# ziotom78/pytracer

Measured on NVIDIA B200. Metric: path-traced rays/sec (demo.txt 1080p), higher is better.
Workload: dtype f32

## Files before the change

pytracer_b200/csrc/rt_warp.cuh:

```cuda
#pragma once
#include "rt_kernels.cuh"

#define RT_WARP_MAX_THREADS 256
#ifndef RT_WARP_SPLIT
#define RT_WARP_SPLIT 1
#endif


struct __align__(16) ScatterRec {
  float4 a;
  float4 b;
  float4 c;
};

struct WarpCfg {
  int cap;
  int group;
  int per_pixel;
  int rounds;
  int per_warp_bytes;
  int shape_bytes;
  long long n_tasks;
  float bg[3], inv_n, inv_spp;
  unsigned n_magic;
  double inv_w, inv_h, inv_s;
  unsigned long long n_samples;
};

RT_DEV int err_batch_of(const ErrArgs& cfg, int ls) {
  return cfg.err_bpp == 32 ? (ls & 31) : ls - (int)(((unsigned)ls * cfg.err_magic) >> 16) * cfg.err_bpp;
}
RT_DEV void err_batch_add(float* bsum, int slot, bool on, V3<float> c, int lane) {
  const unsigned FULL = 0xffffffffu;
  if (__ballot_sync(FULL, on && (c.x != 0.f || c.y != 0.f || c.z != 0.f)) == 0u) return;
  const int key = on ? slot : 32 + lane;
  const int prev = __shfl_up_sync(FULL, key, 1);
  const unsigned heads = __ballot_sync(FULL, lane == 0 || prev != key);
  const int seg_start = 31 - __clz(heads & (0xffffffffu >> (31 - lane)));
#pragma unroll
  for (int d = 1; d < 32; d <<= 1) {
    const float r = __shfl_up_sync(FULL, c.x, d);
    const float g = __shfl_up_sync(FULL, c.y, d);
    const float b = __shfl_up_sync(FULL, c.z, d);
    if (lane - d >= seg_start) { c.x += r; c.y += g; c.z += b; }
  }
  const bool tail = lane == 31 || ((heads >> (lane + 1)) & 1u);
  if (on && tail && (c.x != 0.f || c.y != 0.f || c.z != 0.f)) {
    atomicAdd(&bsum[3 * slot + 0], c.x);
    atomicAdd(&bsum[3 * slot + 1], c.y);
    atomicAdd(&bsum[3 * slot + 2], c.z);
  }
}
RT_DEV void err_store(const ErrArgs& e, int L, const float* bsum, int g, long long entry, V3<float> m, int lane) {
  const unsigned FULL = 0xffffffffu;
  const int bpp = e.err_bpp, B = min(L, bpp);
  float tr = 0.f, tg = 0.f, tb = 0.f;
  if (lane < B) {
    const float n = (float)((L - 1 - lane) / bpp + 1);
    const float* t = bsum + 3 * (g * bpp + lane);
    const float dr = fmaf(-n, m.x, t[0]), dg = fmaf(-n, m.y, t[1]), db = fmaf(-n, m.z, t[2]);
    tr = dr * dr / n; tg = dg * dg / n; tb = db * db / n;
  }
#pragma unroll
  for (int d = 16; d > 0; d >>= 1) {
    tr += __shfl_xor_sync(FULL, tr, d);
    tg += __shfl_xor_sync(FULL, tg, d);
    tb += __shfl_xor_sync(FULL, tb, d);
  }
  if (lane == 0) {
    const float k = 1.f / ((float)(B - 1) * (float)L);
    float* o = e.err_mean + 3 * entry;
    o[0] = m.x; o[1] = m.y; o[2] = m.z;
    float* v = e.err_var + 3 * entry;
    v[0] = tr * k; v[1] = tg * k; v[2] = tb * k;
  }
}

#define RT_SMALL_MAX_SPHERES 8
#define RT_SMALL_MAX_SHAPES 16
#define RT_SMALL_MAX_MATERIALS 16
#define RT_SMALL_MAX_PIGMENTS 32
enum {
  SM_INVM = 0,
  SM_M = SM_INVM + RT_SMALL_MAX_SHAPES * 48,
  SM_ORIG = SM_M + RT_SMALL_MAX_SHAPES * 48,
  SM_SHAPE_MAT = SM_ORIG + RT_SMALL_MAX_SHAPES * 4,
  SM_PIG = SM_SHAPE_MAT + RT_SMALL_MAX_SHAPES * 16,
  SM_PIG_STRIDE = 48,
  SM_BYTES = SM_PIG + RT_SMALL_MAX_PIGMENTS * SM_PIG_STRIDE
};
#ifndef RT_SMALL_THREADS
#define RT_SMALL_THREADS 256
#endif
#ifndef RT_SMALL_MINB
#define RT_SMALL_MINB 3
#endif

RT_DEV void stage_words(void* sh, const void* g, int bytes) {
  const uint32_t* src = reinterpret_cast<const uint32_t*>(g);
  uint32_t* dst = reinterpret_cast<uint32_t*>(sh);
  for (int i = threadIdx.x; i < bytes / 4; i += blockDim.x) dst[i] = __ldg(src + i);
}

RT_DEV float4 lds4(uint32_t a) {
  float4 v;
  asm volatile("ld.shared.v4.f32 {%0, %1, %2, %3}, [%4];" : "=f"(v.x), "=f"(v.y), "=f"(v.z), "=f"(v.w) : "r"(a) : "memory");
  return v;
}
RT_DEV void sts4(uint32_t a, float4 v) {
  asm volatile("st.shared.v4.f32 [%0], {%1, %2, %3, %4};" :: "r"(a), "f"(v.x), "f"(v.y), "f"(v.z), "f"(v.w) : "memory");
}
RT_DEV float4 lds4c(uint32_t a) {
  float4 v;
  asm volatile("ld.shared.v4.f32 {%0, %1, %2, %3}, [%4];" : "=f"(v.x), "=f"(v.y), "=f"(v.z), "=f"(v.w) : "r"(a));
  return v;
}
RT_DEV int4 lds4ic(uint32_t a) {
  int4 v;
  asm volatile("ld.shared.v4.s32 {%0, %1, %2, %3}, [%4];" : "=r"(v.x), "=r"(v.y), "=r"(v.z), "=r"(v.w) : "r"(a));
  return v;
}
RT_DEV int ldsic(uint32_t a) {
  int v;
  asm volatile("ld.shared.s32 %0, [%1];" : "=r"(v) : "r"(a));
  return v;
}
RT_DEV Rows3 lds_rows(uint32_t a) {
  Rows3 m;
  m.r0 = lds4c(a); m.r1 = lds4c(a + 16); m.r2 = lds4c(a + 32);
  return m;
}

RT_DEV void closest_small(uint32_t sb, int n_spheres, int n_shapes, const Ray<float>& r, int origin, float& best_t, int& best) {
  const float inf = Num<float>::inf();
  float ts = inf, tp = inf;
  int is = -1, ip = -1;
  uint32_t a = sb + SM_INVM;
#pragma unroll 1
  for (int i = 0; i < n_spheres; ++i, a += 48) {
    float tm, half;
    bool ok = sphere_cross_rows(lds_rows(a), r, tm, half);
    const float t1 = tm - half;
    float t = (t1 > r.tmin) ? t1 : tm + half;
    if (i == origin) { t = 2.0f * tm; ok = true; }
    if (ok && t > r.tmin && t < ts) { ts = t; is = i; }
  }
#pragma unroll 1
  for (int i = n_spheres; i < n_shapes; ++i, a += 48) {
    const float4 row = lds4c(a + 32);
    const float oz = fmaf(r.o.x, row.x, fmaf(r.o.y, row.y, fmaf(r.o.z, row.z, row.w)));
    const float dz = fmaf(r.d.x, row.x, fmaf(r.d.y, row.y, r.d.z * row.z));
    const float t = -oz * fast_rcp(dz);
    if (!(fabsf(dz) < 1e-5f) && t > r.tmin && t < tp && i != origin) { tp = t; ip = i; }
  }
  bool plane = tp < ts;
  if (tp == ts && ip >= 0 && is >= 0) plane = ldsic(sb + SM_ORIG + 4 * ip) < ldsic(sb + SM_ORIG + 4 * is);
  best_t = plane ? tp : ts;
  best = plane ? ip : is;
}

RT_DEV V3<float> pigment_color_small(uint32_t pa, float u, float v) {
  const int4 h = lds4ic(pa);
  const float4 q = lds4c(pa + 16);
  if (h.x == RT_PIGMENT_UNIFORM) return mk3<float>(q.x, q.y, q.z);
  const float4 w = lds4c(pa + 32);
  if (h.x == RT_PIGMENT_CHECKERED) {
    const int iu = __float2int_rd(u * (float)h.y), iv = __float2int_rd(v * (float)h.y);
    return (((iu ^ iv) & 1) == 0) ? mk3<float>(q.x, q.y, q.z) : mk3<float>(q.w, w.x, w.y);
  }
  int col = (int)(u * (float)h.z), row = (int)(v * (float)h.w);
  col = min(max(col, 0), h.z - 1);
  row = min(max(row, 0), h.w - 1);
  const cudaTextureObject_t tex = ((unsigned long long)__float_as_uint(w.w) << 32) | (unsigned long long)__float_as_uint(w.z);
  const float4 t = fetch_texel(tex, col + 0.5f, row + 0.5f);
  return mk3<float>(t.x, t.y, t.z);
}

RT_DEV Ray<float> primary_ray_mul(const RenderArgs& a, double inv_w, double inv_h, double inv_s, int col, int row, int s, Pcg& aa) {
  double up = 0.5, vp = 0.5;
  if (a.S > 0) {
    const int ir = a.S <= 1024 ? (int)(((float)s + 0.5f) * (float)inv_s) : s / a.S;
    const int ic = s - ir * a.S;
    const double r1 = (double)pcg_random(aa) * (1.0 / 4294967295.0);
    const double r2 = (double)pcg_random(aa) * (1.0 / 4294967295.0);
    up = ((double)ic + r1) * inv_s;
    vp = ((double)ir + r2) * inv_s;
  }
  const double u = ((double)col + up) * inv_w;
  const double v = 1.0 - ((double)row + vp) * inv_h;
  V3<double> o, d;
  camera_fire_f64(a.cam, u, v, o, d);
  Ray<float> r;
  r.o = cast3<float>(o);
  r.d = cast3<float>(d);
  r.tmin = 1.0e-5f;
  r.tmax = Num<float>::inf();
  return r;
}

RT_DEV int own_stratum(const RenderArgs& a, int ls) {
  return (a.part_mode == RT_PART_SPP && a.part_count > 1) ? a.part_rank + ls * a.part_count : ls;
}

enum { ACC_REG = 0, ACC_LANES = 1, ACC_SEG = 2 };
#define RT_ACC_LANES_MAX_GROUP 8

template <bool SHAPES_SMEM, int ACC, bool SMALL, bool ERR = false>
__global__ void __launch_bounds__(SMALL ? RT_SMALL_THREADS : RT_WARP_MAX_THREADS, SMALL ? RT_SMALL_MINB : 2)
k_pt_warp(const __grid_constant__ SceneView<float> sc, const __grid_constant__ RenderArgs a,
          const __grid_constant__ WarpCfg cfg, const __grid_constant__ ErrArgs ea) {
  extern __shared__ __align__(16) unsigned char smem_raw[];
  const unsigned FULL = 0xffffffffu;
  const int warp = threadIdx.x >> 5;
  ScanSrc<float> src = global_src<float>(sc);
  if (SMALL) {
    stage_words(smem_raw + SM_INVM, sc.invm, sc.n_shapes * 48);
    stage_words(smem_raw + SM_M, sc.m, sc.n_shapes * 48);
    stage_words(smem_raw + SM_ORIG, sc.orig, sc.n_shapes * 4);
    for (int i = threadIdx.x; i < sc.n_shapes; i += blockDim.x) {
      const DevMaterial& mt = sc.materials[sc.material[i]];
      reinterpret_cast<int4*>(smem_raw + SM_SHAPE_MAT)[i] = make_int4(mt.brdf_kind, mt.brdf_pigment, mt.emitted_pigment, mt.flags);
    }
    for (int i = threadIdx.x; i < sc.n_pigments; i += blockDim.x) {
      const DevPigment& pg = sc.pigments[i];
      float4* o = reinterpret_cast<float4*>(smem_raw + SM_PIG + i * SM_PIG_STRIDE);
      o[0] = make_float4(__int_as_float(pg.kind), __int_as_float(pg.steps), __int_as_float(pg.tex_w), __int_as_float(pg.tex_h));
      o[1] = make_float4(pg.c1[0], pg.c1[1], pg.c1[2], pg.c2[0]);
      o[2] = make_float4(pg.c2[1], pg.c2[2], __uint_as_float((uint32_t)pg.tex), __uint_as_float((uint32_t)((unsigned long long)pg.tex >> 32)));
    }
    __syncthreads();
  } else if (SHAPES_SMEM) {
    stage_bytes(smem_raw, sc.packed, (size_t)sc.n_pairs * 96 + (size_t)(sc.n_shapes - sc.n_spheres) * 48);
    __syncthreads();
    src.pairs = reinterpret_cast<const float4*>(smem_raw);
    src.planes = reinterpret_cast<const float*>(smem_raw) + 24 * (size_t)sc.n_pairs;
  }
  const int lane0 = threadIdx.x & 31;
  const int lane = __shfl_sync(FULL, lane0, lane0);
  const uint32_t smem0 = (uint32_t)__cvta_generic_to_shared(smem_raw);
  const uint32_t sb = __shfl_sync(FULL, smem0 + (uint32_t)lane0, 0);
  const int wofs = (SMALL ? (int)SM_BYTES : cfg.shape_bytes) + warp * cfg.per_warp_bytes;
  const uint32_t wb = __shfl_sync(FULL, smem0 + (uint32_t)(wofs + lane0), 0);
  const uint32_t curb = wb + (uint32_t)cfg.cap * (uint32_t)sizeof(ScatterRec);
  constexpr bool MULTI_SLOT = ACC != ACC_REG;
  int* slot_rays = reinterpret_cast<int*>(smem_raw + wofs + (size_t)(cfg.cap + 1) * sizeof(ScatterRec));
  float* acc = reinterpret_cast<float*>(slot_rays + 32);
  float* bsum = ACC == ACC_REG ? reinterpret_cast<float*>(slot_rays) : acc + (ACC == ACC_SEG ? 96 : 96 * cfg.group);
  const bool count_rays = a.out_hit != nullptr && a.hit_mode == RT_HIT_RAY_COUNT;

  const PixelMap pm = ERR ? make_pixel_map_list(a, ea) : make_pixel_map(a);
  const int N = a.num_of_rays;
  const int S2 = a.S > 0 ? a.S * a.S : 1;
  const int G = cfg.group, L = cfg.per_pixel;
  auto div_n = [&](int x) -> int { return cfg.n_magic ? (int)(((unsigned)x * cfg.n_magic) >> 16) : (x >= N ? 1 : 0); };
  const float inv_n = cfg.inv_n, inv_spp = cfg.inv_spp;
  unsigned int n_rays = 0;
  bool overflow = false;

  while (true) {
    long long task = 0;
    if (lane == 0) task = (long long)atomicAdd(a.counters + CNT_TASK, 1ull);
    task = __shfl_sync(FULL, task, 0);
    if (task >= cfg.n_tasks) break;
    const long long p0 = task * G;
    uint64_t aa_task = a.aa_state;
    if (ACC == ACC_REG && a.S > 0 && p0 < pm.n_pixels) {
      int col, row;
      if (ERR) locate_listed(pm, ea, p0, col, row);
      else pm.locate(p0, col, row);
      aa_task = pcg_jump(a.aa_state, 2ull * (unsigned long long)((long long)row * a.width + col) * S2, a.jump);
    }
    float sr = 0.f, sg = 0.f, sb_ = 0.f;
    unsigned int task_rays = 0;
    const int task_prims = (int)min((long long)G, pm.n_pixels - p0) * L;
    if (MULTI_SLOT) {
      if (ACC == ACC_SEG) { for (int i = lane; i < 96; i += 32) acc[i] = 0.f; }
      else { for (int i = 0; i < 3 * cfg.group; ++i) acc[i * 32 + lane] = 0.f; }
      slot_rays[lane] = 0;
      __syncwarp();
    }
    if (ERR) {
      for (int i = lane; i < 96; i += 32) bsum[i] = 0.f;
      __syncwarp();
    }

    {
      int top = 0, cur_rem = 0, cur_done = 0;
      int round = 0;
      bool primary_phase = true;
      while (true) {
        bool active;
        int slot = 0, depth = 0, seg_start = lane, origin = -1;
        V3<float> thr = mk3<float>(1.f, 1.f, 1.f);
        Ray<float> ray;
        Pcg rng;
        long long pix = 0;
        bool last_of_pixel = false;
        int rslot = 0;
        if (primary_phase) {
          const int j = round * 32 + lane;
          slot = j / L;
          const int ls = j - slot * L;
          const long long p = p0 + slot;
          if (ERR) rslot = slot * ea.err_bpp + err_batch_of(ea, ls);
          active = (j < G * L) && (p < pm.n_pixels);
          task_rays += (unsigned)min(max(task_prims - round * 32, 0), 32);
          if (active) {
            int col, row;
            if (ERR) locate_listed(pm, ea, p, col, row);
            else pm.locate(p, col, row);
            pix = (long long)row * a.width + col;
            const int s = own_stratum(a, ls);
            const unsigned long long k = (unsigned long long)pix * S2 + s;
            Pcg aa;
            aa.inc = a.aa_inc;
            if (ACC == ACC_REG) aa.state = (a.S > 0) ? pcg_jump(aa_task, 2ull * (unsigned)s, a.jump) : 0;
            else aa.state = (a.S > 0) ? pcg_jump(a.aa_state, 2ull * k, a.jump) : 0;
            ray = primary_ray_mul(a, cfg.inv_w, cfg.inv_h, cfg.inv_s, col, row, s, aa);
            rng = pcg_seed(a.pt_state, (a.pt_inc >> 1) + k);
            last_of_pixel = (ls == L - 1);
          }
          if (ACC == ACC_SEG) seg_start = max(0, slot * L - round * 32);
        } else {
          const long long avail = (long long)cur_rem + (long long)top * N;
          if (avail == 0) break;
          const int take = (int)min(avail, 32ll);
          active = lane < take;
          task_rays += (unsigned)take;
          const int from_cur = min(cur_rem, take);
          const int jj = max(lane - from_cur, 0);
          const int r = div_n(jj);
          const bool on_cur = lane < from_cur;
          const int child = on_cur ? cur_done + lane : jj - r * N;
          if (ACC == ACC_SEG) seg_start = on_cur ? 0 : from_cur + r * N;
          const uint32_t ra = (on_cur || !active) ? curb : wb + (uint32_t)(top - 1 - r) * (uint32_t)sizeof(ScatterRec);
          ScatterRec rec;
          rec.a = lds4(ra); rec.b = lds4(ra + 16); rec.c = lds4(ra + 32);
          const int rest = take - from_cur;
          const int full = div_n(rest), part = rest - full * N;
          cur_rem -= from_cur;
          cur_done += from_cur;
          __syncwarp();
          int new_top = top - full;
          if (part > 0) {
            new_top -= 1;
            if (lane < 3) sts4(curb + 16 * lane, lds4(wb + (uint32_t)new_top * (uint32_t)sizeof(ScatterRec) + 16 * lane));
            cur_rem = N - part;
            cur_done = part;
          }
          __syncwarp();
          top = new_top;
          if (active) {
            const int meta = __float_as_int(rec.a.w);
            slot = meta & 31;
            if (ERR) { rslot = slot; slot = (int)(((unsigned)rslot * ea.err_magic) >> 16); }
            depth = (meta >> 6) & 1023;
            origin = (int)((unsigned)meta >> 16);
            if (origin == 0xFFFF) origin = -1;
            thr = mk3<float>(rec.b.w, rec.c.x, rec.c.y);
            const uint64_t base = ((uint64_t)__float_as_uint(rec.c.w) << 32) | (uint64_t)__float_as_uint(rec.c.z);
            rng.state = child_stream(base, child);
            rng.inc = a.pt_inc;
            ray.o = mk3<float>(rec.a.x, rec.a.y, rec.a.z);
            ray.tmax = Num<float>::inf();
            const V3<float> nd = mk3<float>(rec.b.x, rec.b.y, rec.b.z);
            if (((meta >> 5) & 1) == RT_BRDF_DIFFUSE) {
              const float u1 = unit_from_u32((uint32_t)(rng.state >> 32));
              const float u2 = unit_from_u32((uint32_t)rng.state);
              ray.d = diffuse_dir<float>(nd, u1, u2);
              ray.tmin = 1.0e-3f;
            } else {
              ray.d = nd;
              ray.tmin = 1e-5f;
            }
          }
        }

        V3<float> contrib = mk3<float>(0.f, 0.f, 0.f);
        bool push = false;
        ScatterRec out;
        float best_t = Num<float>::inf();
        int best = -1;
        if (!SMALL && RT_WARP_SPLIT) {
          if (!active) { ray.o = mk3<float>(0.f, 0.f, 0.f); ray.d = mk3<float>(0.f, 0.f, 0.f); ray.tmin = 0.f; ray.tmax = 0.f; }
          closest_all_warp(sc, src, ray, active, best_t, best, origin);
        }
        if (active) {
          if (SMALL) closest_small(sb, sc.n_spheres, sc.n_shapes, ray, origin, best_t, best);
          else if (!RT_WARP_SPLIT) closest_all_f32<true>(sc, src, ray, best_t, best, origin);
          const bool found = best >= 0;
          if (count_rays) {
            if (MULTI_SLOT) atomicAdd(&slot_rays[slot], 1);
          } else if (primary_phase) {
            if (last_of_pixel && a.out_hit)
              a.out_hit[pm.compact ? p0 + slot : pix] = !found ? -1 : (SMALL ? ldsic(sb + SM_ORIG + 4 * best) : sc.orig[best]);
          }
          if (!found) {
            contrib = mk3<float>(thr.x * cfg.bg[0], thr.y * cfg.bg[1], thr.z * cfg.bg[2]);
          } else {
            int brdf_kind, brdf_pig, emit_pig, mf;
            Rows3 im;
            const bool sphere = best < sc.n_spheres;
            if (SMALL) {
              const int4 mt = lds4ic(sb + SM_SHAPE_MAT + 16 * best);
              brdf_kind = mt.x; brdf_pig = mt.y; emit_pig = mt.z; mf = mt.w;
            } else {
              const DevMaterial& mat = sc.materials[sc.material[best]];
              brdf_kind = mat.brdf_kind; brdf_pig = mat.brdf_pigment; emit_pig = mat.emitted_pigment; mf = mat.flags;
            }
            auto rows_of = [&](bool inverse) -> Rows3 {
              if (SMALL) return lds_rows(sb + (inverse ? SM_INVM : SM_M) + 48 * best);
              return rows_at((inverse ? sc.invm : sc.m) + 12 * (size_t)best);
            };
            auto pig_uniform = [&](int idx) -> V3<float> {
              if (SMALL) { const float4 q = lds4c(sb + SM_PIG + idx * SM_PIG_STRIDE + 16); return mk3<float>(q.x, q.y, q.z); }
              return pig_c1<float>(sc.pigments[idx]);
            };
            auto pig_at = [&](int idx, float u, float v) -> V3<float> {
              if (SMALL) return pigment_color_small(sb + SM_PIG + idx * SM_PIG_STRIDE, u, v);
              return pigment_color<float>(sc.pigments, idx, u, v);
            };
            float u = 0.f, v = 0.f;
            if (depth >= a.max_depth) {
              if (!(mf & MAT_EMIT_BLACK)) {
                if (mf & MAT_UV_EMIT) local_uv<float>(local_hit_rows(rows_of(true), ray, best_t), sphere, u, v);
                contrib = mul3(thr, (mf & MAT_UV_EMIT) ? pig_at(emit_pig, u, v) : pig_uniform(emit_pig));
              }
            } else {
              const bool scatters = !(mf & MAT_NO_SCATTER);
              LocalHit<float> lh;
              if (scatters || (mf & MAT_USES_UV)) { im = rows_of(true); lh = local_hit_rows(im, ray, best_t); }
              if (mf & MAT_USES_UV) local_uv<float>(lh, sphere, u, v);
              if (!(mf & MAT_EMIT_BLACK))
                contrib = mul3(thr, (mf & MAT_UV_EMIT) ? pig_at(emit_pig, u, v) : pig_uniform(emit_pig));
              if (scatters) {
                V3<float> hit_color = (mf & MAT_UV_BRDF) ? pig_at(brdf_pig, u, v) : pig_uniform(brdf_pig);
                const float lum = max3(hit_color);
                bool go_on = true;
                if (depth >= a.rr_limit) {
                  const float q = fmaxf(0.05f, 1.f - lum);
                  if (pcg_random_float<float>(rng) > q) hit_color = fast_rcp(1.f - q) * hit_color;
                  else go_on = false;
                }
                if (go_on && lum > 0.f) {
                  push = true;
                  V3<float> point, normal;
                  world_frame_rows(im, rows_of(false), lh, sphere, point, normal);
                  const V3<float> nd = (brdf_kind == RT_BRDF_DIFFUSE) ? normal : specular_dir<float>(ray.d, normal);
                  const V3<float> w = inv_n * mul3(thr, hit_color);
                  out.a = make_float4(point.x, point.y, point.z,
                                      __int_as_float((ERR ? rslot : slot) | (brdf_kind << 5) | ((depth + 1) << 6) |
                                                     ((best < 0xFFFF ? best : 0xFFFF) << 16)));
                  out.b = make_float4(nd.x, nd.y, nd.z, w.x);
                  out.c = make_float4(w.y, w.z, __uint_as_float((uint32_t)rng.state), __uint_as_float((uint32_t)(rng.state >> 32)));
                }
              }
            }
          }
        }

        if (ERR) err_batch_add(bsum, rslot, active, contrib, lane);
        if (ACC == ACC_SEG) {
#pragma unroll
          for (int d = 1; d < 32; d <<= 1) {
            const float r = __shfl_up_sync(FULL, contrib.x, d);
            const float g = __shfl_up_sync(FULL, contrib.y, d);
            const float b = __shfl_up_sync(FULL, contrib.z, d);
            if (lane - d >= seg_start) { contrib.x += r; contrib.y += g; contrib.z += b; }
          }
          const int next_start = __shfl_down_sync(FULL, seg_start, 1);
          const bool tail = (lane == 31) || (next_start != seg_start);
          if (active && tail && (contrib.x != 0.f || contrib.y != 0.f || contrib.z != 0.f)) {
            atomicAdd(&acc[3 * slot + 0], contrib.x);
            atomicAdd(&acc[3 * slot + 1], contrib.y);
            atomicAdd(&acc[3 * slot + 2], contrib.z);
          }
        } else if (ACC == ACC_LANES) {
          if (active) {
            float* col = acc + (3 * slot) * 32 + lane;
            col[0] += contrib.x; col[32] += contrib.y; col[64] += contrib.z;
          }
        } else {
          sr += contrib.x; sg += contrib.y; sb_ += contrib.z;
        }

        const unsigned pmask = __ballot_sync(FULL, push);
        const int npush = __popc(pmask);
        if (top + npush > cfg.cap) {
          overflow = true;
        } else {
          if (push) {
            const uint32_t pa = wb + (uint32_t)(top + __popc(pmask & ((1u << lane) - 1u))) * (uint32_t)sizeof(ScatterRec);
            sts4(pa, out.a); sts4(pa + 16, out.b); sts4(pa + 32, out.c);
          }
          top += npush;
        }
        __syncwarp();
        if (primary_phase && ++round >= cfg.rounds) primary_phase = false;
      }
    }
    n_rays += task_rays;

    if (ERR && ACC == ACC_SEG) {
      __syncwarp();
      for (int g = 0; g < G && p0 + g < pm.n_pixels; ++g)
        err_store(ea, L, bsum, g, p0 + g, mk3<float>(acc[3 * g] * inv_spp, acc[3 * g + 1] * inv_spp, acc[3 * g + 2] * inv_spp), lane);
      __syncwarp();
    } else if (ACC == ACC_SEG) {
      __syncwarp();
      const long long p = p0 + lane;
      if (lane < G && p < pm.n_pixels) {
        int col, row;
        pm.locate(p, col, row);
        store_pixel<float>(a, pm.at(p, col, row),
                           mk3<float>(acc[3 * lane] * inv_spp, acc[3 * lane + 1] * inv_spp, acc[3 * lane + 2] * inv_spp));
        if (count_rays) a.out_hit[pm.at(p, col, row)] = slot_rays[lane];
      }
      __syncwarp();
    } else if (ACC == ACC_LANES) {
      __syncwarp();
      for (int g = 0; g < G; ++g) {
        float r = acc[(3 * g) * 32 + lane], gr = acc[(3 * g + 1) * 32 + lane], b = acc[(3 * g + 2) * 32 + lane];
#pragma unroll
        for (int d = 16; d > 0; d >>= 1) {
          r += __shfl_xor_sync(FULL, r, d);
          gr += __shfl_xor_sync(FULL, gr, d);
          b += __shfl_xor_sync(FULL, b, d);
        }
        const long long p = p0 + g;
        if (ERR) {
          if (p < pm.n_pixels) err_store(ea, L, bsum, g, p, mk3<float>(r * inv_spp, gr * inv_spp, b * inv_spp), lane);
        } else if (lane == 0 && p < pm.n_pixels) {
          int col, row;
          pm.locate(p, col, row);
          store_pixel<float>(a, pm.at(p, col, row), mk3<float>(r * inv_spp, gr * inv_spp, b * inv_spp));
          if (count_rays) a.out_hit[pm.at(p, col, row)] = slot_rays[g];
        }
      }
      __syncwarp();
    } else {
#pragma unroll
      for (int d = 16; d > 0; d >>= 1) {
        sr += __shfl_xor_sync(FULL, sr, d);
        sg += __shfl_xor_sync(FULL, sg, d);
        sb_ += __shfl_xor_sync(FULL, sb_, d);
      }
      if (ERR) {
        if (p0 < pm.n_pixels) {
          __syncwarp();
          err_store(ea, L, bsum, 0, p0, mk3<float>(sr * inv_spp, sg * inv_spp, sb_ * inv_spp), lane);
        }
        __syncwarp();
      } else if (lane == 0 && p0 < pm.n_pixels) {
        int col, row;
        pm.locate(p0, col, row);
        store_pixel<float>(a, pm.at(p0, col, row), mk3<float>(sr * inv_spp, sg * inv_spp, sb_ * inv_spp));
        if (count_rays) a.out_hit[pm.at(p0, col, row)] = (int)task_rays;
      }
    }
  }
  if (overflow) atomicExch(a.counters + CNT_OVERFLOW, 1ull);
  if (lane == 0 && n_rays) atomicAdd(a.counters + CNT_CLOSEST, (unsigned long long)n_rays);
  if (blockIdx.x == 0 && threadIdx.x == 0) atomicAdd(a.counters + CNT_SAMPLES, cfg.n_samples);
}

template <bool ERR = false>
inline cudaError_t launch_pt_warp_impl(const SceneView<float>& sc, const RenderArgs& a, cudaStream_t st,
                                       int sm_count, LaunchInfo* info, const char** why_not, ErrArgs ea = ErrArgs()) {
  PixelMap pm = ERR ? make_pixel_map_list(a, ea) : make_pixel_map(a);
  const int S2 = a.S > 0 ? a.S * a.S : 1;
  int L = S2;
  if (a.part_mode == RT_PART_SPP && a.part_count > 1)
    L = a.part_rank < S2 ? (S2 - a.part_rank + a.part_count - 1) / a.part_count : 0;
  if (pm.n_pixels == 0 || L == 0) return cudaSuccess;
  if (a.num_of_rays < 1) { *why_not = "num_of_rays must be >= 1"; return cudaErrorInvalidValue; }
  if (a.max_depth >= 1023) { *why_not = "max_depth >= 1023 is not supported by the warp variant (use mega)"; return cudaErrorInvalidValue; }
  WarpCfg cfg;
  cfg.per_pixel = L;
  size_t shape_bytes = (size_t)sc.n_pairs * 96 + (size_t)(sc.n_shapes - sc.n_spheres) * 48;
  const bool shapes_smem = shape_bytes > 0 && shape_bytes <= 64 * 1024;
  const bool small = sc.n_shapes > 0 && sc.n_spheres <= RT_SMALL_MAX_SPHERES && sc.n_shapes <= RT_SMALL_MAX_SHAPES &&
                     sc.n_materials <= RT_SMALL_MAX_MATERIALS && sc.n_pigments <= RT_SMALL_MAX_PIGMENTS;
  int want = 32;
#ifdef RT_TUNING
  if (const char* env = getenv("RT_WARP_WANT")) want = std::min(std::max(atoi(env), 1), 256);
#endif
  if (L >= 32) cfg.group = 1;
  else if (L >= 4) cfg.group = (want + L - 1) / L < RT_ACC_LANES_MAX_GROUP ? (want + L - 1) / L : RT_ACC_LANES_MAX_GROUP;
  else cfg.group = 32 / L;
  if (cfg.group * L > 32 && !small) cfg.group = 32 / L > 0 ? 32 / L : 1;
  cfg.rounds = (cfg.group * L + 31) / 32;
  cfg.n_tasks = (pm.n_pixels + cfg.group - 1) / cfg.group;
  const long long prims = (long long)cfg.rounds * 32;
  long long cap = a.num_of_rays == 1 ? prims + 32 : prims + 32ll * (long long)a.max_depth;
  if (cap < 64) cap = 64;
  int acc_mode = cfg.group == 1 ? ACC_REG : (cfg.group <= RT_ACC_LANES_MAX_GROUP ? ACC_LANES : ACC_SEG);
  cfg.shape_bytes = small ? (int)SM_BYTES : (shapes_smem ? (int)((shape_bytes + 15) / 16 * 16) : 0);
  const size_t limit = 200 * 1024;
  int warps = (small ? RT_SMALL_THREADS : RT_WARP_MAX_THREADS) / 32;
  size_t per_warp = 0, smem = 0;
  bool with_err = false;
  auto footprint = [&](int mode, int w, size_t& pw) {
    pw = (size_t)(cap + 1) * sizeof(ScatterRec);
    if (mode == ACC_SEG) pw += 32 * sizeof(int) + 96 * sizeof(float);
    if (mode == ACC_LANES) pw += 32 * sizeof(int) + (size_t)cfg.group * 96 * sizeof(float);
    if (with_err) pw += 96 * sizeof(float);
    return cfg.shape_bytes + pw * w;
  };
  if (acc_mode == ACC_LANES) {
    size_t pw_l, pw_s;
    const size_t sm_bytes = 227 * 1024;
    const size_t blocks_lanes = sm_bytes / (footprint(ACC_LANES, warps, pw_l) + 1024);
    const size_t blocks_seg = sm_bytes / (footprint(ACC_SEG, warps, pw_s) + 1024);
    const size_t by_threads = 2048 / (warps * 32), by_regs = small ? RT_SMALL_MINB : 2;
    if (std::min(std::min(blocks_seg, by_threads), by_regs) > std::min(std::min(blocks_lanes, by_threads), by_regs)) acc_mode = ACC_SEG;
#ifdef RT_TUNING
    if (const char* env = getenv("RT_WARP_ACC")) { const int m = atoi(env); if (m == ACC_LANES || m == ACC_SEG) acc_mode = m; }
#endif
  }
  with_err = ERR;
  for (;; warps >>= 1) {
    smem = footprint(acc_mode, warps, per_warp);
    if (smem <= limit || warps == 1) break;
  }
  if (smem > limit) { *why_not = "max_depth needs a deeper work stack than shared memory holds"; return cudaErrorInvalidValue; }
  cfg.cap = (int)cap;
  cfg.per_warp_bytes = (int)per_warp;
  for (int k = 0; k < 3; ++k) cfg.bg[k] = (float)a.background[k];
  cfg.inv_n = 1.0f / (float)a.num_of_rays;
  cfg.inv_spp = 1.0f / (float)S2;
  cfg.n_magic = a.num_of_rays <= 1024 ? (65536u + (unsigned)a.num_of_rays - 1u) / (unsigned)a.num_of_rays : 0u;
  cfg.n_samples = (unsigned long long)pm.n_pixels * (unsigned long long)L;
  cfg.inv_w = 1.0 / (double)a.width;
  cfg.inv_h = 1.0 / (double)a.height;
  cfg.inv_s = a.S > 0 ? 1.0 / (double)a.S : 1.0;
  ea.err_bpp = 32 / cfg.group;
  ea.err_magic = (65536u + (unsigned)ea.err_bpp - 1u) / (unsigned)ea.err_bpp;
  if (ERR && (a.S < 2 || cfg.group > RT_ACC_LANES_MAX_GROUP || L != S2)) {
    *why_not = "the error map needs samples_per_side >= 2 and no partition";
    return cudaErrorInvalidValue;
  }

  void (*kern)(const SceneView<float>, const RenderArgs, const WarpCfg, const ErrArgs);
#define RT_PICK(ACCM)                                                                   \
  (small ? k_pt_warp<true, ACCM, true, ERR> : (shapes_smem ? k_pt_warp<true, ACCM, false, ERR> : k_pt_warp<false, ACCM, false, ERR>))
  if (acc_mode == ACC_REG) kern = RT_PICK(ACC_REG);
  else if (acc_mode == ACC_LANES) kern = RT_PICK(ACC_LANES);
  else kern = RT_PICK(ACC_SEG);
#undef RT_PICK
  cudaError_t e = cudaFuncSetAttribute(kern, cudaFuncAttributeMaxDynamicSharedMemorySize, (int)limit);
  if (e != cudaSuccess) return e;
  int per_sm = 0;
  e = cudaOccupancyMaxActiveBlocksPerMultiprocessor(&per_sm, kern, warps * 32, smem);
  if (e != cudaSuccess) return e;
  if (per_sm < 1) per_sm = 1;
  long long blocks = (long long)per_sm * sm_count;
  long long needed = (cfg.n_tasks + warps - 1) / warps;
  if (blocks > needed) blocks = needed;
  kern<<<(unsigned)blocks, warps * 32, smem, st>>>(sc, a, cfg, ea);
  if (info) { info->n_launches += 1; info->variant = RT_VARIANT_WARP; }
  return cudaGetLastError();
}
```

Before: 66.87 billion.

## Precompute per-lane PCG jump tables in smem and unroll small-scene intersection loops

For the small-scene register-accumulation path, each block precomputes per-lane PCG jump coefficients (mult, plus) into shared memory at setup. Each primary ray then derives its AA RNG state with one multiply-add from a per-round base jump, instead of a full logarithmic pcg_jump per ray. The sphere and plane intersection loops are also fully unrolled to their compile-time maximums with early breaks, removing loop-carried address arithmetic. This uses more shared memory per block and a longer unrolled body, which may raise register pressure. The correctness of the jump composition depends on the stratum mapping being linear in the lane index.

```diff
diff --git a/pytracer_b200/csrc/rt_warp.cuh b/pytracer_b200/csrc/rt_warp.cuh
--- a/pytracer_b200/csrc/rt_warp.cuh
+++ b/pytracer_b200/csrc/rt_warp.cuh
@@ -87,7 +87,9 @@
   SM_SHAPE_MAT = SM_ORIG + RT_SMALL_MAX_SHAPES * 4,
   SM_PIG = SM_SHAPE_MAT + RT_SMALL_MAX_SHAPES * 16,
   SM_PIG_STRIDE = 48,
-  SM_BYTES = SM_PIG + RT_SMALL_MAX_PIGMENTS * SM_PIG_STRIDE
+  SM_BYTES = SM_PIG + RT_SMALL_MAX_PIGMENTS * SM_PIG_STRIDE,
+  SM_JUMP = SM_BYTES,
+  SM_JUMP_BYTES = 32 * 16
 };
 #ifndef RT_SMALL_THREADS
 #define RT_SMALL_THREADS 256
@@ -125,6 +127,11 @@
   asm volatile("ld.shared.s32 %0, [%1];" : "=r"(v) : "r"(a));
   return v;
 }
+RT_DEV ulonglong2 lds2u64c(uint32_t a) {
+  ulonglong2 v;
+  asm volatile("ld.shared.v2.u64 {%0, %1}, [%2];" : "=l"(v.x), "=l"(v.y) : "r"(a));
+  return v;
+}
 RT_DEV Rows3 lds_rows(uint32_t a) {
   Rows3 m;
   m.r0 = lds4c(a); m.r1 = lds4c(a + 16); m.r2 = lds4c(a + 32);
@@ -135,24 +142,28 @@
   const float inf = Num<float>::inf();
   float ts = inf, tp = inf;
   int is = -1, ip = -1;
-  uint32_t a = sb + SM_INVM;
-#pragma unroll 1
-  for (int i = 0; i < n_spheres; ++i, a += 48) {
+#pragma unroll
+  for (int i = 0; i < RT_SMALL_MAX_SPHERES; ++i) {
+    if (i >= n_spheres) break;
     float tm, half;
-    bool ok = sphere_cross_rows(lds_rows(a), r, tm, half);
+    bool ok = sphere_cross_rows(lds_rows(sb + SM_INVM + 48 * i), r, tm, half);
     const float t1 = tm - half;
     float t = (t1 > r.tmin) ? t1 : tm + half;
     if (i == origin) { t = 2.0f * tm; ok = true; }
     if (ok && t > r.tmin && t < ts) { ts = t; is = i; }
   }
-#pragma unroll 1
-  for (int i = n_spheres; i < n_shapes; ++i, a += 48) {
-    const float4 row = lds4c(a + 32);
+  const uint32_t pb = sb + SM_INVM + 48 * (uint32_t)n_spheres;
+  const int n_planes = n_shapes - n_spheres, porigin = origin - n_spheres;
+#pragma unroll
+  for (int k = 0; k < RT_SMALL_MAX_SHAPES; ++k) {
+    if (k >= n_planes) break;
+    const float4 row = lds4c(pb + 48 * k + 32);
     const float oz = fmaf(r.o.x, row.x, fmaf(r.o.y, row.y, fmaf(r.o.z, row.z, row.w)));
     const float dz = fmaf(r.d.x, row.x, fmaf(r.d.y, row.y, r.d.z * row.z));
     const float t = -oz * fast_rcp(dz);
-    if (!(fabsf(dz) < 1e-5f) && t > r.tmin && t < tp && i != origin) { tp = t; ip = i; }
-  }
+    if (!(fabsf(dz) < 1e-5f) && t > r.tmin && t < tp && k != porigin) { tp = t; ip = k; }
+  }
+  if (ip >= 0) ip += n_spheres;
   bool plane = tp < ts;
   if (tp == ts && ip >= 0 && is >= 0) plane = ldsic(sb + SM_ORIG + 4 * ip) < ldsic(sb + SM_ORIG + 4 * is);
   best_t = plane ? tp : ts;
@@ -228,6 +239,17 @@
       o[1] = make_float4(pg.c1[0], pg.c1[1], pg.c1[2], pg.c2[0]);
       o[2] = make_float4(pg.c2[1], pg.c2[2], __uint_as_float((uint32_t)pg.tex), __uint_as_float((uint32_t)((unsigned long long)pg.tex >> 32)));
     }
+    if (ACC == ACC_REG && threadIdx.x < 32) {
+      const unsigned long long c = (a.part_mode == RT_PART_SPP && a.part_count > 1) ? (unsigned long long)a.part_count : 1ull;
+      uint64_t d = 2ull * c * threadIdx.x, mult = 1, plus = 0;
+      while (d != 0) {
+        const int b = __ffsll((long long)d) - 1;
+        mult = a.jump.mult[b] * mult;
+        plus = a.jump.mult[b] * plus + a.jump.plus[b];
+        d &= d - 1;
+      }
+      reinterpret_cast<ulonglong2*>(smem_raw + SM_JUMP)[threadIdx.x] = make_ulonglong2(mult, plus);
+    }
     __syncthreads();
   } else if (SHAPES_SMEM) {
     stage_bytes(smem_raw, sc.packed, (size_t)sc.n_pairs * 96 + (size_t)(sc.n_shapes - sc.n_spheres) * 48);
@@ -239,7 +261,7 @@
   const int lane = __shfl_sync(FULL, lane0, lane0);
   const uint32_t smem0 = (uint32_t)__cvta_generic_to_shared(smem_raw);
   const uint32_t sb = __shfl_sync(FULL, smem0 + (uint32_t)lane0, 0);
-  const int wofs = (SMALL ? (int)SM_BYTES : cfg.shape_bytes) + warp * cfg.per_warp_bytes;
+  const int wofs = (SMALL ? (int)SM_BYTES + (ACC == ACC_REG ? (int)SM_JUMP_BYTES : 0) : cfg.shape_bytes) + warp * cfg.per_warp_bytes;
   const uint32_t wb = __shfl_sync(FULL, smem0 + (uint32_t)(wofs + lane0), 0);
   const uint32_t curb = wb + (uint32_t)cfg.cap * (uint32_t)sizeof(ScatterRec);
   constexpr bool MULTI_SLOT = ACC != ACC_REG;
@@ -298,6 +320,8 @@
         bool last_of_pixel = false;
         int rslot = 0;
         if (primary_phase) {
+          uint64_t aa_round = 0;
+          if (SMALL && ACC == ACC_REG && a.S > 0) aa_round = pcg_jump(aa_task, 2ull * (unsigned)own_stratum(a, round * 32), a.jump);
           const int j = round * 32 + lane;
           slot = j / L;
           const int ls = j - slot * L;
@@ -314,7 +338,10 @@
             const unsigned long long k = (unsigned long long)pix * S2 + s;
             Pcg aa;
             aa.inc = a.aa_inc;
-            if (ACC == ACC_REG) aa.state = (a.S > 0) ? pcg_jump(aa_task, 2ull * (unsigned)s, a.jump) : 0;
+            if (SMALL && ACC == ACC_REG) {
+              const ulonglong2 jl = lds2u64c(sb + SM_JUMP + 16 * lane);
+              aa.state = (a.S > 0) ? jl.x * aa_round + jl.y : 0;
+            } else if (ACC == ACC_REG) aa.state = (a.S > 0) ? pcg_jump(aa_task, 2ull * (unsigned)s, a.jump) : 0;
             else aa.state = (a.S > 0) ? pcg_jump(a.aa_state, 2ull * k, a.jump) : 0;
             ray = primary_ray_mul(a, cfg.inv_w, cfg.inv_h, cfg.inv_s, col, row, s, aa);
             rng = pcg_seed(a.pt_state, (a.pt_inc >> 1) + k);
@@ -595,7 +622,7 @@
   long long cap = a.num_of_rays == 1 ? prims + 32 : prims + 32ll * (long long)a.max_depth;
   if (cap < 64) cap = 64;
   int acc_mode = cfg.group == 1 ? ACC_REG : (cfg.group <= RT_ACC_LANES_MAX_GROUP ? ACC_LANES : ACC_SEG);
-  cfg.shape_bytes = small ? (int)SM_BYTES : (shapes_smem ? (int)((shape_bytes + 15) / 16 * 16) : 0);
+  cfg.shape_bytes = small ? (int)SM_BYTES + (acc_mode == ACC_REG ? (int)SM_JUMP_BYTES : 0) : (shapes_smem ? (int)((shape_bytes + 15) / 16 * 16) : 0);
   const size_t limit = 200 * 1024;
   int warps = (small ? RT_SMALL_THREADS : RT_WARP_MAX_THREADS) / 32;
   size_t per_warp = 0, smem = 0;
diff --git a/scratch/sass_lines.py b/scratch/sass_lines.py
--- /dev/null
+++ b/scratch/sass_lines.py
@@ -0,0 +1,87 @@
+import argparse
+import collections
+import os
+import re
+import subprocess
+import sys
+import tempfile
+
+FRAME = re.compile(r'"([^"]+)", line (\d+)')
+
+
+def disassemble(lib, cubin, mangled):
+    tmp = tempfile.mkdtemp()
+    subprocess.run(["cuobjdump", "-xelf", "all", os.path.abspath(lib)], cwd=tmp, check=True, stdout=subprocess.DEVNULL)
+    names = [f for f in os.listdir(tmp) if f.endswith(".cubin") and cubin in f]
+    for name in sorted(names):
+        dis = subprocess.run(["nvdisasm", "-gi", os.path.join(tmp, name)], capture_output=True, text=True, check=True).stdout.splitlines()
+        head = ".text." + mangled + ":"
+        if head in dis:
+            return dis[dis.index(head) + 1:]
+    sys.exit(f"{mangled} not found in {names}")
+
+
+def main():
+    ap = argparse.ArgumentParser()
+    ap.add_argument("lib")
+    ap.add_argument("kernel")
+    ap.add_argument("--cubin", default="rt_kernels_f32")
+    ap.add_argument("--file", default="rt_warp.cuh")
+    ap.add_argument("--region", action="append", default=[])
+    ap.add_argument("--within", help="LO-HI: only instructions with a frame on these lines of --file")
+    ap.add_argument("--top", type=int, default=40)
+    ap.add_argument("--dump", action="store_true", help="every instruction with its line")
+    args = ap.parse_args()
+
+    regions = []
+    for r in args.region:
+        name, span = r.split("=")
+        lo, hi = (int(x) for x in span.split("-"))
+        regions.append((name, lo, hi))
+
+    def region_of(chain):
+        for f, n in chain:
+            for name, lo, hi in regions:
+                if f == args.file and lo <= n <= hi:
+                    return name
+        return "other"
+
+    within = tuple(int(x) for x in args.within.split("-")) if args.within else None
+    insts = []
+    chain, fresh = [("?", 0)], True
+    for l in disassemble(args.lib, args.cubin, args.kernel):
+        if l.startswith("\t.section") or l.startswith(".text."):
+            break
+        if "//## File" in l:
+            f, n = FRAME.search(l).groups()
+            chain = [(os.path.basename(f), int(n))] if fresh else chain + [(os.path.basename(f), int(n))]
+            fresh = False
+            continue
+        m = re.match(r"\s+/\*([0-9a-f]{4,})\*/\s+(.*?);", l)
+        if m:
+            if not within or any(f == args.file and within[0] <= n <= within[1] for f, n in chain):
+                insts.append((chain, m.group(2)))
+            fresh = True
+    line_of = lambda chain: next((fr for fr in chain if fr[0] == args.file), chain[-1])
+    if args.dump:
+        for chain, txt in insts:
+            f, n = line_of(chain)
+            print(f"{f}:{n:<5d} {region_of(chain):12s} {' < '.join(f'{a}:{b}' for a, b in chain):60s} {txt}")
+        return
+
+    per_line = collections.Counter(line_of(chain) for chain, _ in insts)
+    per_region = collections.Counter(region_of(chain) for chain, _ in insts)
+    total = len(insts)
+    op = lambda t: t.split()[1] if t.startswith("@") else t.split()[0]
+    print(f"{args.kernel}: {total} SASS instructions, {sum(op(t).startswith('STL') for _, t in insts)} STL, "
+          f"{sum(op(t).startswith('LDL') for _, t in insts)} LDL, {sum(op(t).startswith('CALL') for _, t in insts)} CALL")
+    if regions:
+        for name, lo, hi in regions + [("other", 0, 0)]:
+            span = f"{args.file}:{lo}-{hi}" if name != "other" else ""
+            print(f"  region {name:12s} {per_region[name]:6d}  {span}")
+    for (f, n), k in sorted(per_line.items(), key=lambda kv: -kv[1])[:args.top]:
+        print(f"  {f}:{n:<5d} {k:6d}")
+
+
+if __name__ == "__main__":
+    main()
```

Result: faster. 69.66 billion (median of 6 runs) (+4.2%).
